# akloetgen/PARA-suite

Hardware: AMD Instinct MI355X
Metric: aligned reads/sec (10Mx50bp PAR-CLIP vs hg19-size genome) on MI355X; SAM bit-exact vs own CPU restatement (parity unpinned) (higher is better)
Workload: dtype u64

## Files before the change

### para-suite_amd/csrc/ps_core.h

```cpp
#pragma once
#include "ps_types.h"

namespace ps {

PS_HD uint32_t ps_popc(uint32_t x)
{
#ifdef __HIP_DEVICE_COMPILE__
    return (uint32_t)__popc(x);
#else
    return (uint32_t)__builtin_popcount(x);
#endif
}
PS_HD uint32_t pfx_mask32(int ns)
{
    return ns >= 32 ? 0xFFFFFFFFu : (ns <= 0 ? 0u : ((1u << ns) - 1u));
}

struct Blk { uint32_t x[16]; };

#ifdef __HIP_DEVICE_COMPILE__
#define PS_AS_GLOBAL(T, p) ((const __attribute__((address_space(1))) T *)(p))
#define PS_AS_GLOBAL_W(T, p) ((__attribute__((address_space(1))) T *)(p))
typedef uint32_t ps_u32x4 __attribute__((ext_vector_type(4)));
#endif

PS_HD int opaque_lane(int v)
{
#ifdef __HIP_DEVICE_COMPILE__
    asm volatile("" : "+v"(v));
#endif
    return v;
}

PS_HD void load_blk(const OccBlock *blocks, uint32_t b, Blk &o)
{
#ifdef __HIP_DEVICE_COMPILE__
    const __attribute__((address_space(1))) ps_u32x4 *p = PS_AS_GLOBAL(ps_u32x4, blocks + b);
    const ps_u32x4 a = p[0], c = p[1], d = p[2], e = p[3];
    o.x[0] = a.x; o.x[1] = a.y; o.x[2] = a.z; o.x[3] = a.w;
    o.x[4] = c.x; o.x[5] = c.y; o.x[6] = c.z; o.x[7] = c.w;
    o.x[8] = d.x; o.x[9] = d.y; o.x[10] = d.z; o.x[11] = d.w;
    o.x[12] = e.x; o.x[13] = e.y; o.x[14] = e.z; o.x[15] = e.w;
#else
    const uint32_t *p = reinterpret_cast<const uint32_t *>(blocks + b);
    for (int j = 0; j < 16; ++j) o.x[j] = p[j];
#endif
}
PS_HD void blk_count4(const Blk &b, int r, uint32_t cnt[4])
{
    uint32_t c1 = 0, c2 = 0, c3 = 0;
    const int q = r >> 5;
    const uint32_t part = (1u << (r & 31)) - 1u;
#pragma unroll
    for (int j = 0; j < 6; ++j) {
        const uint32_t m = j < q ? 0xFFFFFFFFu : (j == q ? part : 0u), lo = b.x[4 + j] & m, hi = b.x[10 + j] & m;
        c3 += ps_popc(lo & hi);
        c2 += ps_popc(hi & ~lo);
        c1 += ps_popc(lo & ~hi);
    }
    cnt[0] = b.x[0] + ((uint32_t)r - c1 - c2 - c3);
    cnt[1] = b.x[1] + c1; cnt[2] = b.x[2] + c2; cnt[3] = b.x[3] + c3;
}
PS_HD uint32_t blk_count1(const Blk &b, int r, int c)
{
    uint32_t n = 0;
    const uint32_t flo = (c & 1) ? 0u : 0xFFFFFFFFu, fhi = (c & 2) ? 0u : 0xFFFFFFFFu;
#pragma unroll
    for (int j = 0; j < 6; ++j) n += ps_popc((b.x[4 + j] ^ flo) & (b.x[10 + j] ^ fhi) & pfx_mask32(r - 32 * j));
    uint32_t base = c == 0 ? b.x[0] : (c == 1 ? b.x[1] : (c == 2 ? b.x[2] : b.x[3]));
    return base + n;
}
PS_HD int blk_sym(const Blk &b, int pos)
{
    uint32_t lo = 0, hi = 0; const int wi = pos >> 5;
#pragma unroll
    for (int j = 0; j < 6; ++j) { lo = (j == wi) ? b.x[4 + j] : lo; hi = (j == wi) ? b.x[10 + j] : hi; }
// ... 96 lines not shown
        uint32_t ok, ol;
        occ_pair1(ix, c.k, c.l, base, ok, ol, st);
        const bwtint l2 = L2_of(ix, base);
        c.k = l2 + ok + 1;
        c.l = l2 + ol;
    }
    if (c.k > c.l || base > 3) { c.k = 0; c.l = ix.seq_len; ++c.bid; }
    uint32_t w = width32(c.k, c.l);
    w_out = w;
    cw_out = cw_pack(c.bid, !first && w == c.prev_w);
    c.prev_w = w;
}

static const int PS_POP_TRIES = 1;
enum { M_FETCH = 0, M_POP = 1, M_EXACT = 2, M_EXPAND = 3, M_EXIT = 4, M_HIT = 5,
       M_GROW = 6 };

struct BtLane {
    int r, mode;
    bwtint k, l;
    int i, score, units, n_mm, n_gapo, n_gape, n_ins, n_del, state, ldp;
    bool have_cur;
    int best_score, max_units, n_aln, n_stack, status;
    unsigned long long best_cnt;
    unsigned long long bm0, bm1;
    uint32_t bump, free_head, iters0;
    uint32_t rn0, rn1;
    int len;
    uint32_t n_phantom;
    uint32_t cap;
    LaneStats st;
};

PS_HD int lm_ncw(int len) { return (len + 1 + 3) >> 2; }
PS_HD int lm_ncsw(int seed_len) { return seed_len > 0 ? (seed_len + 1 + 3) >> 2 : 0; }
PS_HD bool lm_nmask_in_regs(int len) { return len <= 64; }
PS_HD int lm_heads_off(int len, int seed_len) { return 4 * (lm_ncw(len) + lm_ncsw(seed_len) + ((len + 15) >> 4) + (lm_nmask_in_regs(len) ? 0 : ((len + 31) >> 5))); }
PS_HD int lm_bytes(int len, int seed_len, int n_buckets, bool wide)
{
    int n = lm_heads_off(len, seed_len) + (wide ? 0 : 2 * n_buckets);
    n = (n + 3) & ~3;
    if (((n >> 2) & 1) == 0) n += 4;
    return n;
}

static const int PS_JUMP_SLOT_WORDS = 8, PS_JUMP_MAX_LEVELS = 14;
PS_HD uint32_t jump_level_off(int d) { return 0x55555555u & ((1u << (2 * d)) - 1u); }
PS_HD size_t jump_words(int levels) { return (size_t)jump_level_off(levels) * PS_JUMP_SLOT_WORDS; }
PS_HD int jump_levels_for(bwtint seq_len) { int k = 0; while (k < PS_JUMP_MAX_LEVELS && (seq_len >> (2 * k)) >= 48) ++k; return k; }

struct BtHot {
    const OccBlock *blocks; bwtint primary;
    const uint32_t *jump; uint32_t jump_levels;
    uint32_t L2lo[4], L2hi;
    uint32_t s_pk[5], u_pk[5];
    uint32_t p0, p1, p2, p3;
    uint32_t inv_c_min, max_entries, pool_cap, n_reads, big_cap;
    uint32_t c_min;
    PS_HD int len() const { return (int)(p0 & 0xffu); }
    PS_HD int seed_len() const { return (int)((p0 >> 8) & 0xffu); }
    PS_HD int indel_end_skip() const { return (int)((p0 >> 16) & 0xffu); }
    PS_HD int max_del_occ() const { return (int)(p0 >> 24); }
    PS_HD int max_gapo() const { return (int)(p1 & 0xfu); }
    PS_HD int max_gape() const { return (int)((p1 >> 4) & 0xfu); }
    PS_HD bool mode_gape() const { return ((p1 >> 8) & 1u) != 0; }
    PS_HD bool use_seed() const { return ((p1 >> 9) & 1u) != 0; }
    PS_HD bool profile() const { return ((p1 >> 10) & 1u) != 0; }
    PS_HD bool has_big() const { return ((p1 >> 11) & 1u) != 0; }
    PS_HD int seed_units() const { return (int)((p1 >> 12) & 0xfffu); }
    PS_HD int u_tight() const { return (int)(p1 >> 24); }
    PS_HD int s_gapo_ins() const { return (int)(p2 & 0xffu); }
    PS_HD int s_gape() const { return (int)((p2 >> 8) & 0xffu); }
    PS_HD int s_gapo_del() const { return (int)((p2 >> 16) & 0xffu); }
    PS_HD int s_stop() const { return (int)(p2 >> 24); }
    PS_HD int u_gapo_ins() const { return (int)(p3 & 0xffu); }
    PS_HD int u_gape() const { return (int)((p3 >> 8) & 0xffu); }
    PS_HD int u_gapo_del() const { return (int)((p3 >> 16) & 0xffu); }
    PS_HD int n_buckets() const { return (int)(p3 >> 24); }
    PS_HD bwtint L2(int c) const
    { return (bwtint)L2lo[c] | ((bwtint)((L2hi >> c) & 1u) << 32); }
    PS_HD bwtint L2_dyn(int c) const
    { return (bwtint)sel4s(L2lo[0], L2lo[1], L2lo[2], L2lo[3], c) | ((bwtint)((L2hi >> c) & 1u) << 32); }
};
inline bool bt_hot_make(const BtArgs &a, BtHot &h)
{
    const Model &md = a.md;
    h.blocks = a.ix.blocks; h.primary = a.ix.primary; h.L2hi = 0;
    h.jump = a.ix.jump; h.jump_levels = a.ix.jump ? (uint32_t)a.ix.jump_levels : 0u;
    for (int c = 0; c < 4; ++c) { h.L2lo[c] = (uint32_t)a.ix.L2[c]; h.L2hi |= (uint32_t)((a.ix.L2[c] >> 32) & 1ull) << c; }
    h.L2hi |= (uint32_t)((a.ix.seq_len >> 32) & 1ull) << 4;
    for (int c = 0; c < 5; ++c) { h.s_pk[c] = md.s_mm_pk[c]; h.u_pk[c] = md.u_mm_pk[c]; }
    const int seed_units = md.max_seed_diff * md.u_tight;
    const bool ok = a.len >= 0 && a.len <= 255 && md.seed_len >= 0 && md.seed_len <= 255 && md.indel_end_skip >= 0 && md.indel_end_skip <= 255 &&
                    md.max_del_occ >= 0 && md.max_del_occ <= 255 && md.max_gapo >= 0 && md.max_gapo <= 15 && md.max_gape >= 0 && md.max_gape <= 15 &&
                    seed_units >= 0 && seed_units <= 4095 && md.u_tight >= 0 && md.u_tight <= 255 && md.s_stop >= 0 && md.s_stop <= 255 &&
                    md.s_gapo_ins >= 0 && md.s_gapo_ins <= 255 && md.s_gape >= 0 && md.s_gape <= 255 && md.s_gapo_del >= 0 && md.s_gapo_del <= 255 &&
                    md.u_gapo_ins >= 0 && md.u_gapo_ins <= 255 && md.u_gape >= 0 && md.u_gape <= 255 && md.u_gapo_del >= 0 && md.u_gapo_del <= 255 &&
                    md.n_buckets >= 0 && md.n_buckets <= 255 && md.max_entries >= 0 && md.inv_c_min >= 0 && md.max_units <= 255 && a.ix.L2[0] == 0;
    h.p0 = (uint32_t)a.len | ((uint32_t)md.seed_len << 8) | ((uint32_t)md.indel_end_skip << 16) | ((uint32_t)md.max_del_occ << 24);
    h.p1 = (uint32_t)md.max_gapo | ((uint32_t)md.max_gape << 4) | ((md.mode_gape ? 1u : 0u) << 8) | ((md.use_seed ? 1u : 0u) << 9) |
           ((md.profile ? 1u : 0u) << 10) | ((a.n_big ? 1u : 0u) << 11) | ((uint32_t)seed_units << 12) | ((uint32_t)md.u_tight << 24);
    h.p2 = (uint32_t)md.s_gapo_ins | ((uint32_t)md.s_gape << 8) | ((uint32_t)md.s_gapo_del << 16) | ((uint32_t)md.s_stop << 24);
    h.p3 = (uint32_t)md.u_gapo_ins | ((uint32_t)md.u_gape << 8) | ((uint32_t)md.u_gapo_del << 16) | ((uint32_t)md.n_buckets << 24);
    h.c_min = (uint32_t)md.c_min;
    h.inv_c_min = (uint32_t)md.inv_c_min; h.max_entries = (uint32_t)md.max_entries; h.pool_cap = a.pool_cap; h.n_reads = (uint32_t)a.n_reads; h.big_cap = a.big_cap;
    return ok;
}

struct BtMem {
    uint8_t *cw, *csw;
    uint32_t *rb, *rn;
    uint16_t *heads16;
    void *pool;
    uint32_t *heads;
};

PS_HD void bt_mem_bind(BtMem &m, uint8_t *mine, int len, int seed_len)
{
    m.cw = mine; m.csw = mine + 4 * lm_ncw(len);
    m.rb = reinterpret_cast<uint32_t *>(m.csw + 4 * lm_ncsw(seed_len));
    m.rn = m.rb + ((len + 15) >> 4);
    m.heads16 = reinterpret_cast<uint16_t *>(mine + lm_heads_off(len, seed_len));
}
PS_HD int seq_at(const BtMem &m, const BtLane &L, int j, int len, int max_len)
{
    const int p = len - 1 - j;
    const uint32_t b = (m.rb[p >> 4] >> (2 * (p & 15))) & 3u;
    const uint32_t nw = lm_nmask_in_regs(max_len) ? (p < 32 ? L.rn0 : L.rn1) : m.rn[p >> 5];
    return ((nw >> (p & 31)) & 1u) ? 4 : 3 - (int)b;
}

struct Entry16 { uint32_t k, l, a, b; };
static const uint32_t PS_NIL16 = 0xFFFFu;

PS_HD bool bm_test(const BtLane &L, int b) { return (((b & 64) ? L.bm1 : L.bm0) >> (b & 63)) & 1ull; }
PS_HD void bm_set(BtLane &L, int b) { const unsigned long long v = 1ull << (b & 63); if (b & 64) L.bm1 |= v; else L.bm0 |= v; }
PS_HD void bm_clr(BtLane &L, int b) { const unsigned long long v = ~(1ull << (b & 63)); if (b & 64) L.bm1 &= v; else L.bm0 &= v; }
PS_HD int bm_first(const BtLane &L)
{
#ifdef __HIP_DEVICE_COMPILE__
    return L.bm0 ? (__ffsll((unsigned long long)L.bm0) - 1) : (64 + __ffsll((unsigned long long)L.bm1) - 1);
// ... 362 lines not shown
```

### para-suite_amd/csrc/ps_kernels.hip

```cpp
#include <hip/hip_runtime.h>
#include <algorithm>
#include <cstdlib>
#include <stdexcept>
#include <string>
#include "ps_core.h"
#include "ps_narrow.h"
#include "ps_kernels.h"

namespace ps {

static const int PS_Q_CHUNK = 64;
#ifndef PS_BT_WAVES
#define PS_BT_WAVES 4
#endif

__device__ __forceinline__ unsigned long long wave_sum(unsigned long long v)
{
    for (int o = 32; o > 0; o >>= 1) v += __shfl_xor(v, o, 64);
    return v;
}
__device__ __forceinline__ void flush_stats(KStats *ks, const LaneStats &st)
{
    if (!ks) return;
    unsigned long long v[8] = {st.pairs, st.same, st.nodes, st.pushes, st.pops, st.lf, st.iters, st.exact};
// ... 14 lines not shown
    for (int r = (blockIdx.x / roles) * blockDim.x + threadIdx.x; r < a.n_reads; r += stride) {
        WChain C;
        wchain_init(a.ix, C);
        const int len = a.lens ? a.lens[r] : a.len, seed_len = a.seed_len;
        const bool seeded = a.use_seed && len > seed_len;
        uint32_t bw = 0, mw = 0;
        uint32_t cww = 0;
        if (!seed_role) {
#pragma unroll 1
            for (int i = 0; i < len; ++i) {
                int j = len - 1 - i;
                if (i == 0 || (j & 15) == 15) bw = a.bases[(size_t)(j >> 4) * a.n_reads + opaque_lane(r)];
                if (i == 0 || (j & 31) == 31) mw = a.nmask[(size_t)(j >> 5) * a.n_reads + opaque_lane(r)];
                int base = ((mw >> (j & 31)) & 1u) ? 4 : (int)((bw >> (2 * (j & 15))) & 3u);
                uint32_t wv; uint8_t cb;
                wchain_step(a.ix, C, base, wv, cb, i == 0, st);
                a.w[(size_t)i * a.n_reads + opaque_lane(r)] = wv;
                cww |= (uint32_t)cb << (8 * (i & 3));
                if ((i & 3) == 3) { a.cwb[(size_t)(i >> 2) * a.n_reads + opaque_lane(r)] = cww; cww = 0; }
            }
            a.w[(size_t)len * a.n_reads + opaque_lane(r)] = 0;
            cww |= (uint32_t)cw_pack(C.bid + 1, false) << (8 * (len & 3));
            a.cwb[(size_t)(len >> 2) * a.n_reads + opaque_lane(r)] = cww;
        } else if (seeded) {
#pragma unroll 1
            for (int i = 0; i < seed_len; ++i) {
                int js = seed_len - 1 - i;
                if (i == 0 || (js & 15) == 15) bw = a.bases[(size_t)(js >> 4) * a.n_reads + opaque_lane(r)];
                if (i == 0 || (js & 31) == 31) mw = a.nmask[(size_t)(js >> 5) * a.n_reads + opaque_lane(r)];
                int sbase = ((mw >> (js & 31)) & 1u) ? 4 : (int)((bw >> (2 * (js & 15))) & 3u);
                uint32_t swv; uint8_t scb;
                wchain_step(a.ix, C, sbase, swv, scb, i == 0, st);
                cww |= (uint32_t)scb << (8 * (i & 3));
                if ((i & 3) == 3) { a.cswb[(size_t)(i >> 2) * a.n_reads + opaque_lane(r)] = cww; cww = 0; }
            }
            cww |= (uint32_t)cw_pack(C.bid + 1, false) << (8 * (seed_len & 3));
            a.cswb[(size_t)(seed_len >> 2) * a.n_reads + opaque_lane(r)] = cww;
        } else if (a.use_seed) {
            for (int p = 0; p <= (seed_len >> 2); ++p) a.cswb[(size_t)p * a.n_reads + opaque_lane(r)] = 0u;
        }
    }
    flush_stats(a.stats, st);
}

__device__ __forceinline__ uint32_t pin32(uint32_t v) { return (uint32_t)__builtin_amdgcn_readfirstlane((int)v); }
__device__ __forceinline__ unsigned long long pin64(unsigned long long v)
{
    return (unsigned long long)pin32((uint32_t)v) | ((unsigned long long)pin32((uint32_t)(v >> 32)) << 32);
}
__device__ __forceinline__ void pin_hot(BtHot &h, const BtHot &k)
{
    h.blocks = reinterpret_cast<const OccBlock *>(pin64(reinterpret_cast<unsigned long long>(k.blocks)));
    h.primary = pin64(k.primary);
    h.jump = reinterpret_cast<const uint32_t *>(pin64(reinterpret_cast<unsigned long long>(k.jump))); h.jump_levels = pin32(k.jump_levels);
#pragma unroll
    for (int c = 0; c < 4; ++c) h.L2lo[c] = pin32(k.L2lo[c]);
    h.L2hi = pin32(k.L2hi);
#pragma unroll
    for (int c = 0; c < 5; ++c) { h.s_pk[c] = pin32(k.s_pk[c]); h.u_pk[c] = pin32(k.u_pk[c]); }
    h.p0 = pin32(k.p0); h.p1 = pin32(k.p1); h.p2 = pin32(k.p2); h.p3 = pin32(k.p3);
    h.c_min = pin32(k.c_min);
    h.inv_c_min = pin32(k.inv_c_min); h.max_entries = pin32(k.max_entries); h.pool_cap = pin32(k.pool_cap); h.n_reads = pin32(k.n_reads); h.big_cap = pin32(k.big_cap);
}

__global__ void __launch_bounds__(256) k_backtrack_wide(const BtArgs *__restrict__ ap, BtHot hk, int lm_stride)
{
    const BtArgs &a = *ap;
    BtHot h; pin_hot(h, hk);
    uint32_t *const queue = reinterpret_cast<uint32_t *>(pin64(reinterpret_cast<unsigned long long>(a.queue)));
    const uint32_t n_reads = h.n_reads, fetch_min = pin32((uint32_t)a.fetch_min), hit_min = pin32((uint32_t)a.hit_min);
    extern __shared__ __attribute__((aligned(16))) uint8_t smem[];
    const int lane_g = blockIdx.x * blockDim.x + threadIdx.x;
    BtMem m;
    bt_mem_bind(m, smem + (size_t)threadIdx.x * lm_stride, h.len(), h.seed_len());
    m.pool = reinterpret_cast<uint8_t *>(a.pool) + (size_t)lane_g * h.pool_cap * sizeof(Entry);
    m.heads = a.heads + (size_t)lane_g * PS_MAX_BUCKETS;
    BtLane L;
    L.mode = M_FETCH; L.r = 0; L.have_cur = false; L.n_stack = 0; L.status = RS_OK; L.n_aln = 0;
    L.st = {0, 0, 0, 0, 0, 0, 0, 0};
    const int lane = threadIdx.x & 63;
    const unsigned long long lane_lt = (1ull << lane) - 1ull;
    const unsigned long long t_start = wall_clock64();
    int q_next = 0, q_end = 0;
    bool exhausted = false;
    for (;;) {
        const bool want = L.mode == M_FETCH;
        const unsigned long long wmask = __ballot(want), lmask = __ballot(L.mode != M_EXIT), hmask = __ballot(L.mode == M_HIT);
        if (lmask == 0) break;
        const bool stalled = (wmask | hmask) == lmask;
        const bool serve_hit = hmask != 0 && (__popcll(hmask) >= (int)hit_min || stalled);
        int fetch_r = -1;
        if (wmask) {
            const int cnt = __popcll(wmask);
            if (cnt >= (int)fetch_min || stalled) {
                const int rank = __popcll(wmask & lane_lt);
                int served = 0;
                while (served < cnt) {
                    if (q_next == q_end) {
                        if (exhausted) break;
                        unsigned int base = 0;
                        if (lane == 0) base = atomicAdd(queue, (unsigned int)PS_Q_CHUNK);
                        base = (unsigned int)__shfl((int)base, 0, 64);
                        if (base >= n_reads) { exhausted = true; break; }
                        q_next = (int)base;
                        q_end = (int)base + PS_Q_CHUNK < (int)n_reads ? (int)base + PS_Q_CHUNK : (int)n_reads;
                    }
                    const int take = q_end - q_next < cnt - served ? q_end - q_next : cnt - served;
// ... 286 lines not shown
```

### para-suite_amd/csrc/ps_narrow.h

```cpp
#pragma once
#include "ps_core.h"

namespace ps {

PS_HD int nw_i(uint32_t wa) { return (int)(wa & 0xffu); }
PS_HD int nw_ldp(uint32_t wa) { return (int)((wa >> 8) & 0xffu); }
PS_HD int nw_mm(uint32_t wa) { return (int)((wa >> 16) & 0xffu); }
PS_HD int nw_state(uint32_t wa) { return (int)((wa >> 24) & 3u); }
PS_HD int nw_gapo(uint32_t wa) { return (int)((wa >> 26) & 7u); }
PS_HD int nw_gape(uint32_t wa) { return (int)(wa >> 29); }
PS_HD int nw_ins(uint32_t wb) { return (int)(wb & 7u); }
PS_HD int nw_del(uint32_t wb) { return (int)((wb >> 3) & 7u); }
PS_HD uint32_t nw_c(uint32_t wb) { return (wb >> 6) & 7u; }
PS_HD int nw_score(uint32_t wb) { return (int)((wb >> 9) & 0x7fu); }
static const uint32_t NW_KEEP = 0xFCFF0000u;
static const uint32_t NW_C_MASK = 7u << 6;
static const uint32_t NW_ROOT_C = 4u;

PS_HD int nl_mode(uint32_t ctl) { return (int)(ctl & 7u); }
PS_HD uint32_t nl_set_mode(uint32_t ctl, int mode) { return (ctl & ~7u) | (uint32_t)mode; }
static const uint32_t NL_HAVE_CUR = 8u, NL_STATUS = 7u << 4, NL_BIG = 1u << 7;
PS_HD int nl_status(uint32_t ctl) { return (int)((ctl >> 4) & 7u); }
PS_HD uint32_t nl_set_status(uint32_t ctl, int s) { return (ctl & ~NL_STATUS) | ((uint32_t)s << 4); }
PS_HD int nl_n_aln(uint32_t ctl) { return (int)(ctl >> 16); }
// ... 238 lines not shown
    if (nNu > max_units) { nt_finish_read(a, L); return false; }
    L.kr = 0; L.lr = (uint32_t)a.ix.seq_len; L.wa = (uint32_t)len; L.wb = NW_ROOT_C << 6;
    L.ctl |= NL_HAVE_CUR;
    L.nsb = 0; L.bm0 = L.bm1 = 0; L.fh = 0xffffu;
    {
        int e = 255;
        if (a.cap_est) { e = (int)a.est[r] - (a.cap_est - 1); if (e < 0) e = 0; }
        L.n_phantom = (uint32_t)(e + md.u_tight < max_units ? e : 255) << 24;
    }
    nt_heads_init(m, md.n_buckets);
    return true;
}

PS_HD uint32_t nt_slot(NLane &L)
{
    const uint32_t fr = L.fh;
    const bool reuse = fr != 0xffffu;
    const uint32_t idx = reuse ? fr : (L.nsb >> 16);
    L.nsb += reuse ? 1u : 0x10001u;
    L.fh = 0xffffu;
    return idx;
}
PS_HD void nt_push(NLane &L, BtMem &m, uint32_t kr, uint32_t lr, uint32_t wa, uint32_t wb)
{
    const int score = nw_score(wb);
    const uint32_t idx = nt_slot(L);
    const uint32_t next = (uint32_t)m.heads16[score];
    Entry16 e; e.k = kr; e.l = lr; e.a = wa; e.b = wb | (next << 16);
    store16(reinterpret_cast<Entry16 *>(m.pool) + idx, e);
    m.heads16[score] = (uint16_t)idx;
    if (score < 32) L.bm0 |= 1u << score; else L.bm1 |= 1u << (score - 32);
}

template <bool NB32>
PS_HD void nt_pop(NLane &L, BtMem &m)
{
#ifdef __HIP_DEVICE_COMPILE__
    const int b = (NB32 || L.bm0) ? __ffs((int)L.bm0) - 1 : 32 + __ffs((int)L.bm1) - 1;
#else
    const int b = (NB32 || L.bm0) ? __builtin_ctz(L.bm0) : 32 + __builtin_ctz(L.bm1);
#endif
    const uint32_t hd = m.heads16[b];
    Entry16 e;
    load16(reinterpret_cast<const Entry16 *>(m.pool) + hd, e);
    const uint32_t next = e.b >> 16;
    L.fh = hd;
    m.heads16[b] = (uint16_t)next;
    if (next == PS_NIL16) { if (NB32 || b < 32) L.bm0 &= ~(1u << b); else L.bm1 &= ~(1u << (b - 32)); }
    L.kr = e.k; L.lr = e.l; L.wa = e.a; L.wb = e.b & 0xffffu;
    L.nsb -= 1u;
}

template <bool STATS, bool NB32>
PS_HD int nt_head(const BtArgs &a, const BtHot &h, NLane &L, LaneStats &st, BtMem &m, int fetch_r, bool serve_hit)
{
    int mode = nl_mode(L.ctl);
    if (mode == M_EXIT || mode == M_GROW) return 0;
    if (STATS) ++st.iters;
    if (mode == M_HIT) {
        if (!serve_hit) return 0;
        L.ctl = nl_set_mode(L.ctl, M_POP);
        { NLane t = L; nt_hit(a, t, m); L = t; }
        return 0;
    }
    if (mode == M_FETCH) {
        if (fetch_r < 0) return 0;
        if (fetch_r >= (int)h.n_reads) { L.ctl = nl_set_mode(L.ctl, M_EXIT); return 0; }
        { NLane t = L; const bool ok = nt_fetch(a, t, m, fetch_r); L = t; if (!ok) return 0; }
        L.ctl = nl_set_mode(L.ctl, M_POP);
        mode = M_POP;
    }
    if (mode == M_POP) {
        const int n_virtual = nl_n_stack(L) + ((L.ctl & NL_HAVE_CUR) ? 1 : 0);
        if (nl_phantom(L) && (long long)n_virtual + (long long)nl_phantom(L) > (long long)h.max_entries) {
            L.ctl = nl_set_status(L.ctl, RS_OVERFLOW_POOL); nt_finish_read(a, L); return 0;
        }
        if (n_virtual == 0 && nl_est(L) != 255 && nl_n_aln(L.ctl) == 0 && nl_status(L.ctl) == RS_OK) { NLane t = L; nt_restart_without_estimate(a, t, m); L = t; return 0; }
        if (n_virtual == 0 || n_virtual > (int)h.max_entries || nl_status(L.ctl) != RS_OK) { nt_finish_read(a, L); return 0; }
        if (L.ctl & NL_HAVE_CUR) L.ctl &= ~NL_HAVE_CUR;
        else { nt_pop<NB32>(L, m); if (STATS) ++st.pops; }
        L.ctl = nl_set_mode(L.ctl, M_POP);
        const int score = nw_score(L.wb), i1 = nw_i(L.wa);
        if (score > nl_best_score(L) + h.s_stop()) { nt_finish_read(a, L); return 0; }
        const int rem = nl_max_units(L) - nt_units(h, L.wa, L.wb);
        if (rem < 0) return 0;
        const int mleft = (int)(ps_mul24((uint32_t)rem, h.inv_c_min) >> 16);
        if (i1 > 0 && mleft < (int)(m.cw[i1 - 1] & 0x7f)) return 0;
        if (i1 == 0) { L.ctl = nl_set_mode(L.ctl, M_HIT); return 0; }
        const int st_ = nw_state(L.wa);
        mode = (mleft == 0 && (st_ == ST_M || h.mode_gape() || nw_gape(L.wa) == h.max_gape())) ? M_EXACT : M_EXPAND;
    }
    return mode;
}

struct NtStep { uint32_t ck[4], cl[4]; uint32_t cw_i, cw_im1, cs_i, cs_im1; int s, i; bool in_seed, tm, ctm; };

template <bool STATS>
PS_HD void nt_step_occ(const BtHot &h, NLane &L, LaneStats &st, BtMem &m, NtStep &q)
{
    const int len = nl_len(L), max_len = h.len();
    const int i = nw_i(L.wa) - 1;
    q.i = i;
    q.cw_i = m.cw[i]; q.cw_im1 = m.cw[i > 0 ? i - 1 : 0];
    const int ii = i - (len - h.seed_len());
    q.in_seed = h.use_seed() && len > h.seed_len() && ii > 0;
    q.cs_i = q.in_seed ? m.csw[ii] : 0u; q.cs_im1 = q.in_seed ? m.csw[ii - 1] : 0u;
    q.s = nt_seq_at(m, L, i, len, max_len);
    const int depth = nt_depth(len, L.wa, L.wb);
    q.tm = depth < (int)h.jump_levels; q.ctm = depth + 1 < (int)h.jump_levels;
    if (!q.tm) nt_occ<STATS>(h, nw_c(L.wb), L.kr, L.lr, q.ck, q.cl, st);
    else nt_jump(h, depth, L.kr, q.ck, q.cl);
}

template <bool STATS, bool NB32>
PS_HD void nt_tail(const BtHot &h, NLane &L, LaneStats &st, BtMem &m, const NtStep &q, int mode)
{
    const int len = nl_len(L), i = q.i, s = q.s;
    const uint32_t cw_i = q.cw_i, cw_im1 = q.cw_im1, cs_i = q.cs_i, cs_im1 = q.cs_im1;
    const bool in_seed = q.in_seed, tm = q.tm, ctm = q.ctm;
    uint32_t ck[4], cl[4];
#pragma unroll
    for (int c = 0; c < 4; ++c) { ck[c] = q.ck[c]; cl[c] = q.cl[c]; }
    if (mode == M_EXACT) {
        if (STATS) ++st.exact;
        L.ctl = nl_set_mode(L.ctl, M_POP);
        if (s > 3) return;
        const uint32_t ok = sel4(ck, s), ol = sel4(cl, s);
        if (ok >= ol) return;
        L.kr = ctm ? (L.kr << 2) | (uint32_t)s : ok + 1u; L.lr = ctm ? ol - ok : ol; L.wa -= 1u; L.wb = (L.wb & ~NW_C_MASK) | ((uint32_t)s << 6);
        L.ctl = nl_set_mode(L.ctl, i == 0 ? M_HIT : M_EXACT);
        return;
    }
    if (STATS) ++st.nodes;
    const uint32_t cap = (L.ctl & NL_BIG) ? h.big_cap : h.pool_cap;
    if (nl_bump(L) + 9u > cap) {
        if (!(L.ctl & NL_BIG) && h.has_big()) { L.ctl = nl_set_mode(L.ctl, M_GROW); return; }
        L.ctl = nl_set_mode(nl_set_status(L.ctl, cap >= 65535u ? RS_OVERFLOW_DEEP : RS_OVERFLOW_POOL), M_POP); return;
    }
// ... 65 lines not shown
            sc[4 + j] = e_sc + (int)((s_word >> (8 * c)) & 0xffu);
            const bool cand = do_mm && xk[j - 1] < xl[j - 1] && cu <= rem, go = cand && cu <= thr_same;
            gmask |= go ? 1u << (4 + j) : 0u;
            phantom += (cand && !go) ? 1u : 0u;
        }
    }
    const uint32_t n_push = ps_popc(gmask), fr = L.fh;
    const bool reuse = fr != 0xffffu && n_push != 0u;
    const uint32_t slot0 = (L.nsb >> 16) - (reuse ? 1u : 0u);
    L.nsb += n_push + ((n_push - (reuse ? 1u : 0u)) << 16);
    L.fh = n_push ? 0xffffu : fr;
    if (STATS) st.pushes += n_push;
    uint32_t idx[9], raw[9];
#pragma unroll
    for (int j = 0; j < 9; ++j) {
        idx[j] = 0; raw[j] = 0;
        if ((gmask >> j) & 1u) {
            const uint32_t rank = ps_popc(gmask & ((1u << j) - 1u));
            idx[j] = (reuse && rank == 0u) ? fr : slot0 + rank;
            raw[j] = m.heads16[sc[j]];
            m.heads16[sc[j]] = (uint16_t)idx[j];
            if (NB32 || sc[j] < 32) L.bm0 |= 1u << sc[j]; else L.bm1 |= 1u << (sc[j] - 32);
        }
    }
#ifdef __HIP_DEVICE_COMPILE__
    asm volatile("" : "+v"(raw[0]), "+v"(raw[1]), "+v"(raw[2]), "+v"(raw[3]), "+v"(raw[4]), "+v"(raw[5]), "+v"(raw[6]), "+v"(raw[7]), "+v"(raw[8]));
#endif
    Entry16 *const pool = reinterpret_cast<Entry16 *>(m.pool);
#define NT_NEXT(j) (raw[j] << 16)
    if (gmask & 1u) { Entry16 e; e.k = pkr; e.l = plr; e.a = wa_i; e.b = (wb0 + 1u) | ((uint32_t)sc[0] << 9) | NT_NEXT(0); store16(pool + idx[0], e); }
    {
        const uint32_t wb_d = ((wb0 & 0x3fu) + (1u << 3)) | ((uint32_t)sc[1] << 9);
#pragma unroll
        for (int c = 0; c < 4; ++c)
            if ((gmask >> (1 + c)) & 1u) { Entry16 e; e.k = ctm ? (pkr << 2) | (uint32_t)c : ck[c] + 1u; e.l = ctm ? cl[c] - ck[c] : cl[c]; e.a = wa_d; e.b = wb_d | ((uint32_t)c << 6) | NT_NEXT(1 + c); store16(pool + idx[1 + c], e); }
    }
    {
        const uint32_t wa_x = wa_keep + pos2 + (1u << 16), wb_x = wb0 & 0x3fu;
#pragma unroll
        for (int j = 1; j <= 4; ++j) {
            const uint32_t c = (uint32_t)((s + j) & 3);
            if ((gmask >> (4 + j)) & 1u) { Entry16 e; e.k = ctm ? (pkr << 2) | c : xk[j - 1] + 1u; e.l = ctm ? xl[j - 1] - xk[j - 1] : xl[j - 1]; e.a = wa_x; e.b = wb_x | (c << 6) | ((uint32_t)sc[4 + j] << 9) | NT_NEXT(4 + j); store16(pool + idx[4 + j], e); }
        }
    }
#undef NT_NEXT
    L.ctl = nl_set_mode(L.ctl, M_POP);
    if (s < 4 && xk[3] < xl[3]) {
        L.kr = ctm ? (pkr << 2) | (uint32_t)s : xk[3] + 1u; L.lr = ctm ? xl[3] - xk[3] : xl[3]; L.wa = wa_keep + (uint32_t)i; L.wb = (L.wb & ~NW_C_MASK) | ((uint32_t)s << 6);
        L.ctl |= NL_HAVE_CUR;
    }
    L.n_phantom += phantom;
}

template <bool STATS, bool NB32>
PS_HD void nt_iter(const BtArgs &a, const BtHot &h, NLane &L, LaneStats &st, BtMem &m, int fetch_r, bool serve_hit, NtClock *clk = nullptr)
{
    PS_USTAMP(clk, 0);
    const int mode = nt_head<STATS, NB32>(a, h, L, st, m, fetch_r, serve_hit);
    PS_USTAMP(clk, 1);
    NtStep q;
    if (mode) nt_step_occ<STATS>(h, L, st, m, q);
#if defined(PS_STAMPS) && defined(__HIP_DEVICE_COMPILE__)
    if (STATS && clk && mode) asm volatile("" :: "v"(q.ck[0]), "v"(q.cl[0]), "v"(q.ck[3]), "v"(q.cl[3]));
#endif
    PS_USTAMP(clk, 2);
    if (mode) nt_tail<STATS, NB32>(h, L, st, m, q, mode);
    PS_USTAMP(clk, 3);
}

}
```

### para-suite_amd/csrc/ps_search.hip

```cpp
#include <hip/hip_runtime.h>
#include <hipcub/hipcub.hpp>
#include <algorithm>
#include <cstring>
#include <optional>
#include "ps_pipeline.h"
#include "ps_search_plan.h"
#include "ps_dev.h"
#include "ps_par.h"

namespace ps {

__global__ void k_gather_alns(const AlnRec *alns, int aln_cap, const int32_t *n_aln, const uint32_t *off, int n, AlnRec *out)
{
    for (int r = blockIdx.x * blockDim.x + threadIdx.x; r < n; r += gridDim.x * blockDim.x) {
        int m = n_aln[r]; if (m > aln_cap) m = aln_cap;
        for (int j = 0; j < m; ++j) out[off[r] + j] = alns[(size_t)r * aln_cap + j];
    }
}
__global__ void k_clip_counts(const int32_t *n_aln, int aln_cap, int n, uint32_t *out)
{
    for (int r = blockIdx.x * blockDim.x + threadIdx.x; r < n; r += gridDim.x * blockDim.x) { int m = n_aln[r]; out[r] = (uint32_t)(m > aln_cap ? aln_cap : (m < 0 ? 0 : m)); }
}

__global__ void k_order_keys(const uint8_t *est, int n, int cap, uint8_t *key)
// ... 39 lines not shown
        em.n_reads = n; em.len = a.len; em.lens = a.lens; em.units_by_len = a.units_by_len; em.bases = a.bases; em.nmask = a.nmask; em.cwb = a.cwb; em.est = est;
        for (int c = 0; c < 5; ++c) em.s_pk[c] = md.u_mm_pk[c];
        em.inv_c_min = (uint32_t)md.inv_c_min; em.max_units = md.max_units; em.u_tight = md.u_tight;
        em.seed_units = md.max_seed_diff * md.u_tight; em.use_seed = md.use_seed; em.seed_len = md.seed_len;
        em.max_gapo = md.max_gapo; em.indel_end_skip = md.indel_end_skip; em.u_gapo_ins = md.u_gapo_ins; em.u_gapo_del = md.u_gapo_del;
        em.depth = lv + 3; em.rows = (float)a.ix.seq_len; em.log_scale = kn.order_scale;
        em.key = key; em.pred = nullptr;
        launch_effort_model(em, s);
    }
    launch_order_sort(key, n, wk->ws_get<uint32_t>("order_tmp", order_sort_tmp_words(n)), order, s);
    PS_HIP(hipGetLastError());
    t->stop(s);
    a.order = order; a.est = est; a.est_ab = ea.est_ab;
}

static const uint8_t *upload_units_by_len(Batch &b)
{
    uint8_t *tab = b.wk->pin_get<uint8_t>("units_by_len_h", 256), *d_tab = b.wk->ws_get<uint8_t>("units_by_len", 256);
    budget_units_by_len(b.ctx->opt, tab);
    PS_HIP(hipMemcpyAsync(d_tab, tab, 256, hipMemcpyHostToDevice, b.wk->stream));
    return d_tab;
}

static SearchPlan search_stacks(Batch &b, BtArgs &a, const SearchKnobs &kn, int lm)
{
    Ctx *ctx = b.ctx; Work *wk = b.wk; hipStream_t s = wk->stream;
    const SearchPlan p = plan_search(a.n_reads, lm, a.pool_cap, a.wide != 0, ctx->cus, ctx->bt_blocks, kn.max_per_cu, ctx->n_big);
    a.n_lanes = p.lanes;
    a.pool = wk->ws_get<uint8_t>("pool", p.pool_bytes);
    a.heads = a.wide ? wk->ws_get<uint32_t>("heads", p.head_words) : nullptr;
    a.queue = wk->ws_get<uint32_t>("queue", 16);
    PS_HIP(hipMemsetAsync(a.queue, 0, 64, s));
    if (p.n_big) {
        a.big_cap = PS_BIG_CAP; a.n_big = p.n_big;
        a.big_pool = wk->ws_get<uint8_t>("big_pool", p.big_bytes);
        a.big_next = a.queue + 4;
        a.big_busy = wk->ws_get<uint32_t>("big_busy", a.n_big);
        PS_HIP(hipMemsetAsync(a.big_busy, 0, (size_t)a.n_big * 4, s));
    }
    return p;
}

static void run_search(Batch &b, const SearchKnobs &kn, const Model &md, int n, const uint32_t *d_bases, const uint32_t *d_nmask, const int32_t *d_lens,
                       uint32_t pool_cap, int aln_cap, AlnRec *alns, int32_t *n_aln, uint8_t *status, bool first_tier = false)
{
    Ctx *ctx = b.ctx; Work *wk = b.wk; hipStream_t s = wk->stream;
    const int len = md.len;
    const bool wide = launch_is_wide(md, pool_cap);
    BtArgs a; std::memset(&a, 0, sizeof a);
    a.ix = ctx->ix.view; a.md = md; a.n_reads = n; a.len = len; a.lens = d_lens;
    a.bases = d_bases; a.nmask = d_nmask; a.n_bw = (len + 15) / 16; a.n_mw = (len + 31) / 32;
    a.alns = alns; a.aln_cap = aln_cap; a.n_aln = n_aln; a.status = status;
    a.pool_cap = pool_cap; a.wide = wide ? 1 : 0; a.stats = b.d_stats.p + 1; a.fetch_min = kn.fetch_min; a.hit_min = kn.hit_min;
    EventPair t_width; std::optional<EventPair> t_order;
    search_width(b, a, t_width);
    if (d_lens) a.units_by_len = upload_units_by_len(b);
    search_order(b, a, kn, t_order);
    a.cap_est = (first_tier && !wide && a.est && md.profile && kn.cap) ? 1 + kn.cap_bias : 0;
    const int lm = lm_bytes(len, md.seed_len, md.n_buckets, wide);
    const SearchPlan p = search_stacks(b, a, kn, lm);
    if (ctx->want_read_iters) { a.read_iters = wk->ws_get<uint32_t>("riters", (size_t)n * PS_RI_WORDS); PS_HIP(hipMemsetAsync(a.read_iters, 0, (size_t)n * PS_RI_WORDS * 4, s)); }
    EventPair t(s);
    if (!launch_backtrack(a, wk->ws_get<BtArgs>("btargs", 1), wk->pin_get<BtArgs>("btargs_h", 1), p.blocks, lm, s, ctx->want_kstats || ctx->want_read_iters)) throw Error("cost model outside the ranges the search kernel packs (gap/score fields must fit a byte)");
    PS_HIP(hipGetLastError());
    t.stop(s);
    const double ms = t.ms(); b.tm.ms_backtrack += ms; ++b.tm.n_backtrack_launches;
    b.tm.ms_width += t_width.ms();
    if (t_order) b.tm.ms_width += t_order->ms();
    { double t0_ = 0, t1_ = 0; t.span(ctx->ref_event, t0_, t1_); if (b.tm.n_backtrack_launches == 1) b.tm.bt_begin_ms = t0_; b.tm.bt_end_ms = t1_; }
    if (std::getenv("PS_VERBOSE")) std::fprintf(stderr, "[parasuite-hip]   backtrack launch: %d reads x %d bp, stack %u%s, %d lanes, %.1f ms\n", n, len, pool_cap, wide ? " (wide)" : "", p.lanes, ms);
    if (ctx->want_read_iters) { ctx->read_iters.resize((size_t)n * PS_RI_WORDS); PS_HIP(hipMemcpyAsync(ctx->read_iters.data(), a.read_iters, (size_t)n * PS_RI_WORDS * 4, hipMemcpyDeviceToHost, s)); PS_HIP(hipStreamSynchronize(s)); }
}

static void download_alns(Work *wk, int n, int aln_cap, const AlnRec *d_alns, const int32_t *d_n_aln,
                          std::vector<int32_t> &n_aln, std::vector<uint32_t> &off, std::vector<AlnRec> &alns)
{
    hipStream_t s = wk->stream;
    uint32_t *cnt = wk->ws_get<uint32_t>("cnt", n), *d_off = wk->ws_get<uint32_t>("off", (size_t)n + 1);
    hipLaunchKernelGGL(k_clip_counts, dim3((n + 255) / 256), dim3(256), 0, s, d_n_aln, aln_cap, n, cnt);
    size_t tb = 0;
    PS_HIP(hipcub::DeviceScan::ExclusiveSum(nullptr, tb, cnt, d_off, n, s));
    uint8_t *tmp = wk->ws_get<uint8_t>("scan_tmp", tb ? tb : 1);
    PS_HIP(hipcub::DeviceScan::ExclusiveSum(tmp, tb, cnt, d_off, n, s));
    int32_t *p_na = wk->pin_get<int32_t>("dl_n_aln", n); uint32_t *p_off = wk->pin_get<uint32_t>("dl_off", (size_t)n + 1);
    PS_HIP(hipMemcpyAsync(p_na, d_n_aln, (size_t)n * 4, hipMemcpyDeviceToHost, s));
    PS_HIP(hipMemcpyAsync(p_off, d_off, (size_t)n * 4, hipMemcpyDeviceToHost, s));
    PS_HIP(hipStreamSynchronize(s));
    uint32_t last = 0;
    if (n) { int m = p_na[n - 1]; last = p_off[n - 1] + (uint32_t)(m > aln_cap ? aln_cap : (m < 0 ? 0 : m)); }
    p_off[n] = last;
    n_aln.assign(p_na, p_na + n); off.assign(p_off, p_off + n + 1); alns.resize(last);
    if (last) {
        AlnRec *comp = wk->ws_get<AlnRec>("comp", last);
        hipLaunchKernelGGL(k_gather_alns, dim3((n + 255) / 256), dim3(256), 0, s, d_alns, aln_cap, d_n_aln, d_off, n, comp);
        AlnRec *p_al = wk->pin_get<AlnRec>("dl_alns", last);
        PS_HIP(hipMemcpyAsync(p_al, comp, (size_t)last * sizeof(AlnRec), hipMemcpyDeviceToHost, s));
        PS_HIP(hipStreamSynchronize(s));
        std::memcpy(alns.data(), p_al, (size_t)last * sizeof(AlnRec));
    }
}

__global__ void k_classify(const AlnRec *alns, int aln_cap, const int32_t *n_aln, const uint8_t *status, const int32_t *ids,
                           int n, int n_occ, uint8_t *cls_out)
{
    for (int r = blockIdx.x * blockDim.x + threadIdx.x; r < n; r += gridDim.x * blockDim.x) {
        uint8_t c = 0;
// ... 212 lines not shown
```

### para-suite_amd/csrc/ps_search_plan.h

```cpp
#pragma once
#include <algorithm>
#include <cstdint>
#include <cstdlib>
#include "ps_budget.h"
#include "ps_core.h"
#include "ps_error.h"
#include "ps_model.h"

namespace ps {

struct SearchKnobs {
    int order = 1, order_min = 4096, order_restart = 0 , order_wpin = 16, order_cap = 255, order_scale = 8;
    int max_per_cu = PS_SEARCH_WAVES;
    bool cap = true; int cap_bias = 0;
    int fetch_min = 8, hit_min = 1;
};
inline SearchKnobs search_knobs_from_env(int ctx_fetch_min, int ctx_hit_min)
{
    SearchKnobs k; int v = 0;
    k.fetch_min = ctx_fetch_min; k.hit_min = ctx_hit_min;
    if (env_int("PS_ORDER", v)) k.order = v;
    if (env_int("PS_ORDER_MIN", v)) k.order_min = std::max(1, v);
    if (env_int("PS_ORDER_RESTART", v)) k.order_restart = std::max(1, v);
    if (env_int("PS_ORDER_WPIN", v)) k.order_wpin = std::max(1, v);
    if (env_int("PS_ORDER_CAP", v)) k.order_cap = std::max(1, std::min(255, v));
    if (env_int("PS_ORDER_SCALE", v)) k.order_scale = std::max(1, std::min(12, v));
    if (env_int("PS_MAX_PER_CU", v)) k.max_per_cu = v;
    if (env_int("PS_CAP", v)) k.cap = v != 0;
    if (env_int("PS_CAP_BIAS", v)) k.cap_bias = std::max(0, std::min(200, v));
    if (env_int("PS_FETCH_MIN", v)) k.fetch_min = std::max(1, v);
    if (env_int("PS_HIT_MIN", v)) k.hit_min = std::max(1, v);
    return k;
}

struct SearchPlan { int blocks = 0, lanes = 0; size_t pool_bytes = 0, head_words = 0; uint32_t n_big = 0; size_t big_bytes = 0; };
static const uint32_t PS_BIG_CAP = 65535;
inline SearchPlan plan_search(int64_t n_reads, int lm_bytes_per_lane, uint32_t pool_cap, bool wide, int cus, int bt_blocks, int max_per_cu, int n_big)
{
    int per_cu = (int)(PS_CU_LDS / ((size_t)256 * lm_bytes_per_lane));
    if (per_cu < 1) throw Error("read length / score range too large for the per-lane LDS state");
    if (bt_blocks <= 0 && max_per_cu < 1) throw Error("PS_MAX_PER_CU must be at least 1");
    int64_t blocks = std::min<int64_t>(bt_blocks > 0 ? bt_blocks : (int64_t)cus * std::min(per_cu, max_per_cu), (n_reads + 255) / 256);
    const size_t entry = wide ? sizeof(Entry) : sizeof(Entry16), per_lane = (size_t)pool_cap * entry + (wide ? PS_MAX_BUCKETS * 4 : 0);
    const size_t max_lanes = ((size_t)(wide ? 32 : 64) << 30) / per_lane;
    if ((size_t)blocks * 256 > max_lanes) blocks = (int64_t)std::max<size_t>(1, max_lanes / 256);
    SearchPlan p;
    p.blocks = (int)blocks; p.lanes = p.blocks * 256;
    p.pool_bytes = (size_t)p.lanes * pool_cap * entry;
    p.head_words = wide ? (size_t)p.lanes * PS_MAX_BUCKETS : 0;
    if (!wide && pool_cap < PS_BIG_CAP && n_big > 0) {
        p.n_big = (uint32_t)std::min<int64_t>(n_big, std::max<int64_t>(64, n_reads));
        p.big_bytes = (size_t)p.n_big * PS_BIG_CAP * sizeof(Entry16);
    }
    return p;
}
inline SearchPlan plan_search_reserve(uint32_t pool_cap, int cus, int bt_blocks, int n_big)
{
    if (pool_cap > PS_BIG_CAP) return SearchPlan();
    return plan_search(INT32_MAX, (int)PS_SEARCH_LDS_PER_LANE, pool_cap, false, cus, bt_blocks, PS_SEARCH_WAVES, n_big);
}

inline void budget_units_by_len(const Options &o, uint8_t tab[256])
{
    for (int l = 0; l < 256; ++l) { const int u = budget_diffs(o, l) * (o.profile ? o.unit : 1); tab[l] = (uint8_t)(u > 255 ? 255 : u); }
}

}
```

### para-suite_amd/csrc/ps_types.h

```cpp
#pragma once
#include <stdint.h>
#include <stddef.h>

#ifdef __HIPCC__
#define PS_HD __host__ __device__ __forceinline__
#define PS_COLD __host__ __device__ inline __attribute__((noinline))
#else
#define PS_HD inline
#define PS_COLD inline
#endif

namespace ps {

typedef uint64_t bwtint;
static const bwtint PS_MAX_ROWS = (1ull << 33) - 64;

static const int PS_BLK_SYMS = 192;
struct OccBlock { uint32_t cnt[4]; uint32_t sym[12]; };

struct IndexView {
    const OccBlock *blocks;
    const uint32_t *sa;
    const uint32_t *sa_hi;
    const uint8_t  *pac;
// ... 8 lines not shown
};

struct Model {
    uint8_t u_mm[5][4], s_mm[5][4];
    uint32_t u_mm_pk[5], s_mm_pk[5];
    int32_t u_gapo_ins, s_gapo_ins, u_gapo_del, s_gapo_del, u_gape, s_gape;
    int32_t s_stop, u_tight, c_min, inv_c_min , max_units, n_buckets;
    int32_t max_gapo, max_gape, mode_gape, indel_end_skip, max_del_occ, max_entries;
    int32_t seed_len, max_seed_diff, max_top2, use_seed, len, profile;
};
static const int PS_MAX_BUCKETS = 128;
static const int PS_MAX_LEN = 250;

struct Entry {
    bwtint k, l;
    uint16_t score, units;
    uint8_t i, last_diff_pos, n_mm, n_gapo, n_gape, n_ins, n_del, state;
    uint32_t next;
};
static const uint32_t PS_NIL = 0xFFFFFFFFu;
enum { ST_M = 0, ST_I = 1, ST_D = 2 };

struct AlnRec {
    bwtint k, l;
    uint16_t score, units;
    uint8_t n_mm, n_gapo, n_gape, n_ins, n_del, pad[7];
};

enum { RS_OK = 0, RS_OVERFLOW_POOL = 1, RS_OVERFLOW_ALN = 2, RS_BAD_SCORE = 3,
       RS_OVERFLOW_DEEP = 4 };

struct KStats {
    unsigned long long occ_pairs, occ_same_blk, nodes, pushes, pops, lf_steps, iters, exact_steps;
};

static const int PS_RI_WORDS = 20;
struct BtArgs {
    IndexView ix;
    Model md;
    int n_reads, len, n_lanes;
    const int32_t *lens;
    const uint8_t *units_by_len;
    const uint32_t *bases; const uint32_t *nmask; int n_bw, n_mw;
    uint32_t *w; const uint32_t *cwb; const uint32_t *cswb;
    AlnRec *alns; int aln_cap; int32_t *n_aln; uint8_t *status;
    void *pool; uint32_t pool_cap;
    uint32_t *heads;
    int wide;
    uint8_t *big_pool; uint32_t big_cap, n_big; uint32_t *big_busy; uint32_t *big_next;
    uint32_t *queue;
    const int32_t *order;
    const uint8_t *est; const uint16_t *est_ab;
    int cap_est;
    uint32_t *read_iters;
    int hit_min;
    int fetch_min;
    KStats *stats;
};

}
```

Before: 8.854 million.

## Skip multiple exact-match backtracking steps via precomputed jump table lookup

Adds a table-skip path to the narrow backtracking iteration. When the remaining mismatch budget cannot be spent on the next few positions (checked with packed byte-wise comparisons against the cw/csw lower bounds) and no N bases occur there, the k-mer of up to four read bases indexes the precomputed jump table, which gives the SA interval directly and advances the lane several positions at once instead of doing one occ step per base. The intent is fewer Occ block lookups per read. In exchange each iteration does extra bit manipulation and a dependent global load, and the path adds correctness risk for SAM bit-exactness. It can be disabled with PS_SKIP=0 and is off when budget units are large.

```diff
diff --git a/para-suite_amd/csrc/ps_core.h b/para-suite_amd/csrc/ps_core.h
--- a/para-suite_amd/csrc/ps_core.h
+++ b/para-suite_amd/csrc/ps_core.h
@@ -22,6 +22,7 @@
 #define PS_AS_GLOBAL(T, p) ((const __attribute__((address_space(1))) T *)(p))
 #define PS_AS_GLOBAL_W(T, p) ((__attribute__((address_space(1))) T *)(p))
 typedef uint32_t ps_u32x4 __attribute__((ext_vector_type(4)));
+typedef uint32_t ps_u32x2 __attribute__((ext_vector_type(2)));
 #endif
 
 PS_HD int opaque_lane(int v)
@@ -224,6 +225,7 @@
 struct BtHot {
     const OccBlock *blocks; bwtint primary;
     const uint32_t *jump; uint32_t jump_levels;
+    uint32_t skip_levels;
     uint32_t L2lo[4], L2hi;
     uint32_t s_pk[5], u_pk[5];
     uint32_t p0, p1, p2, p3;
@@ -259,6 +261,7 @@
     const Model &md = a.md;
     h.blocks = a.ix.blocks; h.primary = a.ix.primary; h.L2hi = 0;
     h.jump = a.ix.jump; h.jump_levels = a.ix.jump ? (uint32_t)a.ix.jump_levels : 0u;
+    h.skip_levels = (a.no_skip || (((uint32_t)md.max_units * (uint32_t)md.inv_c_min) >> 16) > 127u) ? 0u : h.jump_levels;
     for (int c = 0; c < 4; ++c) { h.L2lo[c] = (uint32_t)a.ix.L2[c]; h.L2hi |= (uint32_t)((a.ix.L2[c] >> 32) & 1ull) << c; }
     h.L2hi |= (uint32_t)((a.ix.seq_len >> 32) & 1ull) << 4;
     for (int c = 0; c < 5; ++c) { h.s_pk[c] = md.s_mm_pk[c]; h.u_pk[c] = md.u_mm_pk[c]; }
diff --git a/para-suite_amd/csrc/ps_kernels.hip b/para-suite_amd/csrc/ps_kernels.hip
--- a/para-suite_amd/csrc/ps_kernels.hip
+++ b/para-suite_amd/csrc/ps_kernels.hip
@@ -90,7 +90,7 @@
 {
     h.blocks = reinterpret_cast<const OccBlock *>(pin64(reinterpret_cast<unsigned long long>(k.blocks)));
     h.primary = pin64(k.primary);
-    h.jump = reinterpret_cast<const uint32_t *>(pin64(reinterpret_cast<unsigned long long>(k.jump))); h.jump_levels = pin32(k.jump_levels);
+    h.jump = reinterpret_cast<const uint32_t *>(pin64(reinterpret_cast<unsigned long long>(k.jump))); h.jump_levels = pin32(k.jump_levels); h.skip_levels = pin32(k.skip_levels);
 #pragma unroll
     for (int c = 0; c < 4; ++c) h.L2lo[c] = pin32(k.L2lo[c]);
     h.L2hi = pin32(k.L2hi);
diff --git a/para-suite_amd/csrc/ps_narrow.h b/para-suite_amd/csrc/ps_narrow.h
--- a/para-suite_amd/csrc/ps_narrow.h
+++ b/para-suite_amd/csrc/ps_narrow.h
@@ -314,9 +314,10 @@
 }
 
 template <bool STATS, bool NB32>
-PS_HD int nt_head(const BtArgs &a, const BtHot &h, NLane &L, LaneStats &st, BtMem &m, int fetch_r, bool serve_hit)
+PS_HD int nt_head(const BtArgs &a, const BtHot &h, NLane &L, LaneStats &st, BtMem &m, int fetch_r, bool serve_hit, int &rem_out)
 {
     int mode = nl_mode(L.ctl);
+    rem_out = 0;
     if (mode == M_EXIT || mode == M_GROW) return 0;
     if (STATS) ++st.iters;
     if (mode == M_HIT) {
@@ -346,6 +347,7 @@
         if (score > nl_best_score(L) + h.s_stop()) { nt_finish_read(a, L); return 0; }
         const int rem = nl_max_units(L) - nt_units(h, L.wa, L.wb);
         if (rem < 0) return 0;
+        rem_out = rem;
         const int mleft = (int)(ps_mul24((uint32_t)rem, h.inv_c_min) >> 16);
         if (i1 > 0 && mleft < (int)(m.cw[i1 - 1] & 0x7f)) return 0;
         if (i1 == 0) { L.ctl = nl_set_mode(L.ctl, M_HIT); return 0; }
@@ -517,14 +519,138 @@
     L.n_phantom += phantom;
 }
 
+#ifndef PS_TABLE_SKIP
+#define PS_TABLE_SKIP 1
+#endif
+static const int NT_SKIP_MAX = 4;
+struct NtSkip { uint32_t ck, cl; };
+static const uint32_t NT_NO_SKIP = 0xFFFFFFFFu;
+
+PS_HD uint32_t nt_bytes_below(uint32_t hi, uint32_t lo, uint32_t e)
+{
+#ifdef __HIP_DEVICE_COMPILE__
+    return __builtin_amdgcn_alignbyte(hi, lo, e & 3u);
+#else
+    const uint32_t sh = 8u * (e & 3u);
+    return sh ? (hi << (32u - sh)) | (lo >> sh) : lo;
+#endif
+}
+PS_HD uint32_t nt_bits_from(uint32_t hi, uint32_t lo, uint32_t sh)
+{
+#ifdef __HIP_DEVICE_COMPILE__
+    return __builtin_amdgcn_alignbit(hi, lo, sh);
+#else
+    return sh ? (hi << (32u - sh)) | (lo >> sh) : lo;
+#endif
+}
+PS_HD uint32_t nt_clz(uint32_t x)
+{
+#ifdef __HIP_DEVICE_COMPILE__
+    return (uint32_t)__clz((int)x);
+#else
+    return x ? (uint32_t)__builtin_clz(x) : 32u;
+#endif
+}
+PS_HD uint32_t nt_brev(uint32_t x)
+{
+#ifdef __HIP_DEVICE_COMPILE__
+    return __brev(x);
+#else
+    x = ((x & 0x55555555u) << 1) | ((x >> 1) & 0x55555555u); x = ((x & 0x33333333u) << 2) | ((x >> 2) & 0x33333333u);
+    x = ((x & 0x0f0f0f0fu) << 4) | ((x >> 4) & 0x0f0f0f0fu); x = ((x & 0x00ff00ffu) << 8) | ((x >> 8) & 0x00ff00ffu);
+    return (x << 16) | (x >> 16);
+#endif
+}
+PS_HD uint32_t nt_ge_key(int v)
+{
+    const uint32_t u = (uint32_t)(v > 128 ? 128 : v);
+#ifdef __HIP_DEVICE_COMPILE__
+    return 0x80808080u - __builtin_amdgcn_perm(u, u, 0u);
+#else
+    return 0x80808080u - u * 0x01010101u;
+#endif
+}
+
+PS_HD int nt_skip(const BtHot &h, NLane &L, const BtMem &m, int mode, int rem, NtSkip &sk)
+{
+    sk.ck = NT_NO_SKIP; sk.cl = 0;
+    const int len = nl_len(L), i1 = nw_i(L.wa);
+    const int d = nt_depth(len, L.wa, L.wb);
+    int t = (int)h.skip_levels - 1 - d;
+    t = t > NT_SKIP_MAX ? NT_SKIP_MAX : t;
+    t = t > i1 - 1 ? i1 - 1 : t;
+    const int mleft = (int)(ps_mul24((uint32_t)rem, h.inv_c_min) >> 16);
+    const uint32_t cap = (L.ctl & NL_BIG) ? h.big_cap : h.pool_cap;
+    if (mode != M_EXPAND || t <= 0 || mleft == 0 || nl_bump(L) + 9u > cap) return mode;
+    const uint32_t e = (uint32_t)(i1 - 1);
+    const uint32_t *cw32 = reinterpret_cast<const uint32_t *>(m.cw);
+    const int w0 = (int)(e >> 2);
+    const uint32_t x0 = cw32[w0], x1 = cw32[w0 > 0 ? w0 - 1 : 0];
+    const int r0 = len - i1;
+    const int qb = r0 >> 4, qb_last = ((len + 15) >> 4) - 1;
+    const uint32_t rb_lo = m.rb[qb], rb_hi = m.rb[qb < qb_last ? qb + 1 : qb_last];
+    uint32_t nlo, nhi;
+    if (lm_nmask_in_regs(h.len())) { const bool up = r0 >= 32; nlo = up ? L.rn1 : L.rn0; nhi = up ? 0u : L.rn1; }
+    else { const int qn = r0 >> 5, qn_last = ((len + 31) >> 5) - 1; nlo = m.rn[qn]; nhi = m.rn[qn < qn_last ? qn + 1 : qn_last]; }
+    const uint32_t sum = (nt_bytes_below(x0, x1, e) & 0x7f7f7f7fu) + nt_ge_key(mleft);
+    uint32_t barren = sum & 0x80808080u;
+    const uint32_t kills = (sum - 0x01010101u) & 0x80808080u;
+    if (h.use_seed()) {
+        const int off = len - h.seed_len(), ii = (int)e - off;
+        const uint32_t vs = (uint32_t)((off > 0 && ii > 0) ? ii : 0);
+        const int e_un = nl_max_units(L) - rem, srem = h.seed_units() - e_un;
+        const int m_seed = srem <= 0 ? 0 : (int)(ps_mul24((uint32_t)srem, h.inv_c_min) >> 16);
+        const uint32_t *cs32 = reinterpret_cast<const uint32_t *>(m.csw);
+        const int s0 = (int)(vs >> 2);
+        const uint32_t y0 = cs32[s0], y1 = cs32[s0 > 0 ? s0 - 1 : 0];
+        const uint32_t valid = vs >= 4u ? 0xFFFFFFFFu : ~(0xFFFFFFFFu >> (8u * vs));
+        barren |= ((nt_bytes_below(y0, y1, vs) & 0x7f7f7f7fu) + nt_ge_key(m_seed)) & valid & 0x80808080u;
+    }
+    const int run = (int)(nt_clz(barren ^ 0x80808080u) >> 3);
+    t = t > run ? run : t;
+    if (t == 0) return mode;
+    const bool dead = (int)(nt_clz(kills) >> 3) < t || (nt_bits_from(nhi, nlo, (uint32_t)(r0 & 31)) & ((1u << t) - 1u)) != 0u;
+    uint32_t y = nt_brev(nt_bits_from(rb_hi, rb_lo, (uint32_t)(2 * (r0 & 15))));
+    y = ((y & 0x55555555u) << 1) | ((y >> 1) & 0x55555555u);
+    const uint32_t sidx = (L.kr << (2 * t)) | (~y >> (32 - 2 * t));
+    const uint32_t c = sidx & 3u;
+    const uint32_t *ps = h.jump + (size_t)((jump_level_off(d + t - 1) + (sidx >> 2)) * (uint32_t)PS_JUMP_SLOT_WORDS + 2u * c);
+#ifdef __HIP_DEVICE_COMPILE__
+    const ps_u32x2 v = *PS_AS_GLOBAL(ps_u32x2, ps);
+    sk.ck = v.x; sk.cl = v.y;
+#else
+    sk.ck = ps[0]; sk.cl = ps[1];
+#endif
+    L.kr = sidx;
+    L.wa = (L.wa & NW_KEEP) + (uint32_t)(i1 - t);
+    L.wb = (L.wb & ~NW_C_MASK) | (c << 6);
+    if (dead) L.ctl = nl_set_mode(L.ctl, M_POP);
+    return dead ? 0 : mode;
+}
+PS_HD int nt_skip_land(NLane &L, const NtSkip &sk, int mode)
+{
+    if (sk.ck == NT_NO_SKIP) return mode;
+    if (sk.ck >= sk.cl) { L.ctl = nl_set_mode(L.ctl, M_POP); return 0; }
+    L.lr = sk.cl - sk.ck;
+    return mode;
+}
+
 template <bool STATS, bool NB32>
 PS_HD void nt_iter(const BtArgs &a, const BtHot &h, NLane &L, LaneStats &st, BtMem &m, int fetch_r, bool serve_hit, NtClock *clk = nullptr)
 {
     PS_USTAMP(clk, 0);
-    const int mode = nt_head<STATS, NB32>(a, h, L, st, m, fetch_r, serve_hit);
+    int rem = 0;
+    int mode = nt_head<STATS, NB32>(a, h, L, st, m, fetch_r, serve_hit, rem);
     PS_USTAMP(clk, 1);
+    NtSkip sk;
+    sk.ck = NT_NO_SKIP;
+    if (PS_TABLE_SKIP && mode) mode = nt_skip(h, L, m, mode, rem, sk);
     NtStep q;
     if (mode) nt_step_occ<STATS>(h, L, st, m, q);
+    if (PS_TABLE_SKIP) mode = nt_skip_land(L, sk, mode);
+#if PS_TABLE_SKIP && defined(__HIP_DEVICE_COMPILE__)
+    asm volatile("" : "+v"(L.kr), "+v"(L.lr), "+v"(L.wa), "+v"(L.wb), "+v"(L.ctl), "+v"(mode));
+#endif
 #if defined(PS_STAMPS) && defined(__HIP_DEVICE_COMPILE__)
     if (STATS && clk && mode) asm volatile("" :: "v"(q.ck[0]), "v"(q.cl[0]), "v"(q.ck[3]), "v"(q.cl[3]));
 #endif
diff --git a/para-suite_amd/csrc/ps_search.hip b/para-suite_amd/csrc/ps_search.hip
--- a/para-suite_amd/csrc/ps_search.hip
+++ b/para-suite_amd/csrc/ps_search.hip
@@ -115,6 +115,7 @@
     a.bases = d_bases; a.nmask = d_nmask; a.n_bw = (len + 15) / 16; a.n_mw = (len + 31) / 32;
     a.alns = alns; a.aln_cap = aln_cap; a.n_aln = n_aln; a.status = status;
     a.pool_cap = pool_cap; a.wide = wide ? 1 : 0; a.stats = b.d_stats.p + 1; a.fetch_min = kn.fetch_min; a.hit_min = kn.hit_min;
+    a.no_skip = kn.skip ? 0 : 1;
     EventPair t_width; std::optional<EventPair> t_order;
     search_width(b, a, t_width);
     if (d_lens) a.units_by_len = upload_units_by_len(b);
diff --git a/para-suite_amd/csrc/ps_search_plan.h b/para-suite_amd/csrc/ps_search_plan.h
--- a/para-suite_amd/csrc/ps_search_plan.h
+++ b/para-suite_amd/csrc/ps_search_plan.h
@@ -13,6 +13,7 @@
     int order = 1, order_min = 4096, order_restart = 0 , order_wpin = 16, order_cap = 255, order_scale = 8;
     int max_per_cu = PS_SEARCH_WAVES;
     bool cap = true; int cap_bias = 0;
+    bool skip = true;
     int fetch_min = 8, hit_min = 1;
 };
 inline SearchKnobs search_knobs_from_env(int ctx_fetch_min, int ctx_hit_min)
@@ -28,6 +29,7 @@
     if (env_int("PS_MAX_PER_CU", v)) k.max_per_cu = v;
     if (env_int("PS_CAP", v)) k.cap = v != 0;
     if (env_int("PS_CAP_BIAS", v)) k.cap_bias = std::max(0, std::min(200, v));
+    if (env_int("PS_SKIP", v)) k.skip = v != 0;
     if (env_int("PS_FETCH_MIN", v)) k.fetch_min = std::max(1, v);
     if (env_int("PS_HIT_MIN", v)) k.hit_min = std::max(1, v);
     return k;
diff --git a/para-suite_amd/csrc/ps_types.h b/para-suite_amd/csrc/ps_types.h
--- a/para-suite_amd/csrc/ps_types.h
+++ b/para-suite_amd/csrc/ps_types.h
@@ -84,6 +84,7 @@
     const int32_t *order;
     const uint8_t *est; const uint16_t *est_ab;
     int cap_est;
+    int no_skip;
     uint32_t *read_iters;
     int hit_min;
     int fetch_min;
```

New measurement: 9.479 million (median of 6 runs). 1.07x the previous value.
